# konstantineder/montecarlo-risk-engine

Measured on AMD Instinct MI355X. Metric: path-steps/sec at 1M paths x 250 steps; PV/CVA rel-error vs CPU ref, higher is better.
Workload: dtype f64

## Files before the change

montecarlo-risk-engine_amd/csrc/kf_lean.hip:

```cpp
#include <cstdlib>
#include <map>
#include <utility>

#include "kf_common.h"

namespace {

template <int NSLOT, int PPL>
__device__ __forceinline__ void lean_date_cva(const FastDateCvaLds* __restrict__ rp, const double (&reg)[PPL][2 * NSLOT], double (&cva)[PPL],
                                              const double* __restrict__ etab)
{
    const mcx_expq_coef ec = mcx_expq_load(mcx_region_zero());
    const FastDateCvaLds r = *rp;
    double xe[2 * PPL], ev[2 * PPL];
#pragma unroll
    for (int q = 0; q < PPL; ++q) {
        xe[2 * q] = fma(r.m_s1, reg[q][FDC_S_REG], fma(r.m_n1, reg[q][FDC_NI_REG], r.m_c0));
        xe[2 * q + 1] = fma(r.c_c1, reg[q][FDC_C_REG], r.c_c0);
    }
    mcx_exp_tab_n<2 * PPL>(xe, ev, etab, ec);
#pragma unroll
    for (int q = 0; q < PPL; ++q) {
        const double x = fma(r.x_d, reg[q][FDC_X_REG], r.x_a);
        double p = 0.0;
        p += fma(fma(r.row0[2], x, r.row0[1]), x, r.row0[0]);
        p += fma(fma(r.row1[2], x, r.row1[1]), x, r.row1[0]);
        const double w = r.m_b * ev[2 * q];
        const double cs = fma(r.c_b, ev[2 * q + 1], r.c_a);
        cva[q] = fma(fmax(p, 0.0), w * (1.0 - cs), cva[q]);
    }
}

template <int PPL>
__device__ __forceinline__ void philox4x32_10_cva(const uint32_t (&path_lo)[PPL], uint32_t path_hi, uint32_t step, uint32_t draw, uint64_t seed,
                                                  uint32_t (&o0)[PPL], uint32_t (&o1)[PPL], uint32_t (&o2)[PPL], uint32_t (&o3)[PPL])
{
    constexpr uint32_t M0 = 0xD2511F53u, M1 = 0xCD9E8D57u, W0 = 0x9E3779B9u, W1 = 0xBB67AE85u;
    uint32_t k0 = (uint32_t)seed, k1 = (uint32_t)(seed >> 32);
    uint32_t c0[PPL], c1[PPL], c2[PPL], c3[PPL];
    const uint64_t s1 = (uint64_t)M1 * step;
    const uint32_t hk = path_hi ^ k0;
    const uint32_t a0 = (uint32_t)(s1 >> 32) ^ hk, a1 = (uint32_t)s1;
    const uint32_t dk = draw ^ k1;
#pragma unroll
    for (int q = 0; q < PPL; ++q) {
        const uint64_t p0 = (uint64_t)M0 * path_lo[q];
        c2[q] = (uint32_t)(p0 >> 32) ^ dk;
        c3[q] = (uint32_t)p0;
    }
    k0 += W0; k1 += W1;
    const uint64_t s0 = (uint64_t)M0 * a0;
#pragma unroll
    for (int q = 0; q < PPL; ++q) {
        const uint64_t p1 = (uint64_t)M1 * c2[q];
        c0[q] = ((uint32_t)(p1 >> 32) ^ k0) ^ a1;
        c2[q] = (c3[q] ^ k1) ^ (uint32_t)(s0 >> 32);
        c1[q] = (uint32_t)p1;
    }
    k0 += W0; k1 += W1;
    const uint32_t x3 = (uint32_t)s0 ^ k1;
#pragma unroll
    for (int q = 0; q < PPL; ++q) {
        const uint64_t p0 = (uint64_t)M0 * c0[q];
        const uint64_t p1 = (uint64_t)M1 * c2[q];
        c0[q] = __builtin_amdgcn_bitop3_b32((uint32_t)(p1 >> 32), c1[q], k0, 0x96);
        c2[q] = (uint32_t)(p0 >> 32) ^ x3;
        c1[q] = (uint32_t)p1; c3[q] = (uint32_t)p0;
    }
    k0 += W0; k1 += W1;
#pragma unroll
    for (int r = 3; r < 10; ++r) {
#pragma unroll
        for (int q = 0; q < PPL; ++q) {
            const uint64_t p0 = (uint64_t)M0 * c0[q];
            const uint64_t p1 = (uint64_t)M1 * c2[q];
            const uint32_t n0 = __builtin_amdgcn_bitop3_b32((uint32_t)(p1 >> 32), c1[q], k0, 0x96);
            const uint32_t n2 = __builtin_amdgcn_bitop3_b32((uint32_t)(p0 >> 32), c3[q], k1, 0x96);
            c1[q] = (uint32_t)p1; c3[q] = (uint32_t)p0; c0[q] = n0; c2[q] = n2;
        }
        k0 += W0; k1 += W1;
    }
#pragma unroll
    for (int q = 0; q < PPL; ++q) { o0[q] = c0[q]; o1[q] = c1[q]; o2[q] = c2[q]; o3[q] = c3[q]; }
}

struct CvaDrawConst {
    double off52;
    double trig_scale;
};
__device__ __forceinline__ CvaDrawConst cva_draw_const_make()
{
    CvaDrawConst c;
    c.off52 = mcx_opaque_v(0x1.0p52 - 0.5); c.trig_scale = mcx_opaque_v(6.28318530717958647692 * 0x1.0p-53);
    return c;
}

template <int PPL, int BMB>
__device__ __forceinline__ bool cva_draw_pairs(uint64_t seed, const uint32_t (&path_lo)[PPL], uint32_t path_hi, uint32_t step, uint32_t draw,
                                               double (&z0)[PPL], double (&z1)[PPL], const double* __restrict__ tab,
                                               const mcx_bm_coef& C, const mcx_bm_vconst& vc, const CvaDrawConst& dc)
{
    static_assert(BMB >= 1 && BMB <= 20, "the funnel shift of the high word is by 11 + BMB < 32 bits");
    constexpr int N = 1 << BMB, LOG_TERMS = mcx_bm_shape<BMB>::LOG_TERMS;
    uint32_t w0[PPL], w1[PPL], w2[PPL], w3[PPL];
    philox4x32_10_cva<PPL>(path_lo, path_hi, step, draw, seed, w0, w1, w2, w3);
    double m[PPL], ed[PPL], ps[PPL], pc[PPL];
    int e[PPL];
    mcx_d2 tc[PPL], sc[PPL];
#pragma unroll
    for (int q = 0; q < PPL; ++q) {
        const double ua = u53(w0[q], w1[q], &vc);
        m[q] = __builtin_amdgcn_frexp_mant(ua);
        e[q] = __builtin_amdgcn_frexp_exp(ua);
        const int jl = (__double2hiint(m[q]) >> (20 - BMB)) & (N - 1);
        tc[q] = ((const mcx_d2*)tab)[jl];
        sc[q] = ((const mcx_d2*)(tab + 2 * N))[(int)(w3[q] >> (32 - BMB))];
    }
    __builtin_amdgcn_sched_barrier(0);
#pragma unroll
    for (int q = 0; q < PPL; ++q) {
        const uint32_t lo = __builtin_amdgcn_alignbit(w3[q], w2[q], 11);
        const uint32_t hi = __builtin_amdgcn_alignbit(0x43300000u >> (21 - BMB), w3[q] << BMB, 11 + BMB);
        const double v = __hiloint2double((int)hi, (int)lo) - dc.off52;
        const double d = fma(v, dc.trig_scale, vc.trig_off);
        const double d2 = d * d;
        double qs, qc;
        if constexpr (mcx_bm_shape<BMB>::TRIG_TERMS == 3) {
            qs = fma(fma(vc.sin_head, d2, C.c[7]), d2, C.c[6]);
            qc = fma(fma(vc.cos_head, d2, C.c[10]), d2, C.c[9]);
        } else {
            qs = fma(vc.sin_head, d2, C.c[6]);
            qc = fma(vc.cos_head, d2, C.c[9]);
        }
        ps[q] = fma(d * d2, qs, d);
        pc[q] = fma(d2, qc, 1.0);
        ed[q] = (double)e[q];
    }
    __builtin_amdgcn_sched_barrier(0);
    uint32_t top = 0;
#pragma unroll
    for (int q = 0; q < PPL; ++q) {
        const double s = fma(m[q], tc[q].x, 2.0);
        double p = vc.log_head;
#pragma unroll
        for (int k = LOG_TERMS - 2; k >= 0; --k) p = fma(p, s, C.c[k]);
        const double r2 = fma(ed[q], -2.0 * 6.93147180559945309417e-01, tc[q].y) + fma(s * s, p, s);
        const double r = mcx_sqrt_gp(r2);
        const double sn = fma(sc[q].x, pc[q], sc[q].y * ps[q]);
        const double cs = fma(-sc[q].x, ps[q], sc[q].y * pc[q]);
        z0[q] = r * cs;
        z1[q] = r * sn;
        top = w1[q] > top ? w1[q] : top;
    }
    return top == 0xffffffffu;
}

#define MCX_LEAN_WAVES 4
template <int NSLOT, int NZ, bool INJECT, int SIG, int PPL, bool SIMULATE, int DK = 0>
__global__ __launch_bounds__(MCX_BLOCK, MCX_LEAN_WAVES) void kf_lean(const FusedArgs)
{
    static_assert(DK == 0 || (SIG == SIG_VAS_CIR_E && SIMULATE && !INJECT), "the cva-date kernel simulates the Vasicek + CIR++ signature");
    constexpr int NREG = 2 * NSLOT;
    constexpr int TILE = MCX_BLOCK * PPL;
    extern __shared__ double lds[];
    KArgs& a0 = kargs_region(0);
    const int n_rec = a0.n_rec;
    const int64_t n = a0.k1.n;
    for (int q = threadIdx.x; q < 9 * n_rec; q += MCX_BLOCK) lds[q] = 0.0;
    FastDateCvaLds* const dlds = (FastDateCvaLds*)(lds + ((9 * n_rec + 1) & ~1));
    if constexpr (DK != 0) {
        const FastDateCva* __restrict__ dc = a0.cva_dates;
        const double* __restrict__ cf = a0.coeffs;
        const int n_dates = a0.n_dates;
        for (int q = threadIdx.x; q < 16 * n_dates; q += MCX_BLOCK) {
            const int t = q >> 4, e = q & 15;
            double v;
            if (e < FDC_HEAD) {
                v = ((const double*)(dc + t))[e];
            } else {
                const int off = e < FDC_HEAD + 3 ? dc[t].coeff_off0 : dc[t].coeff_off1;
                v = off >= 0 ? cf[off + (e - FDC_HEAD) % 3] : 0.0;
            }
            ((double*)dlds)[q] = v;
        }
    }
    constexpr int BMB = SIG == SIG_VAS_CIR_E ? 10 : 7;
    constexpr int BM = (INJECT || !SIMULATE) ? 0 : MCX_BM_LDS_DOUBLES_B(BMB);
    __shared__ double tab_lds[BM + MCX_EXP_LDS_DOUBLES];
    const double* tab = nullptr;
    const double* etab = tab_lds + BM;
    mcx_exp_tab_load(tab_lds + BM);
    if (BM) { mcx_bm_load<BMB>(tab_lds); tab = tab_lds; }
    __syncthreads();
    const int64_t tiles = (n + TILE - 1) / TILE;
    double n_block = 0.0;

    for (int64_t tile = blockIdx.x; tile < tiles; tile += gridDim.x) {
        const bool first_tile = tile == (int64_t)blockIdx.x;
        int64_t i[PPL];
        bool live[PPL];
        uint64_t path[PPL];
        double reg[PPL][NREG];
        double cfs[PPL], cva[PPL];
        int est[PPL];
        int n_init, n_steps;
        {
            KArgs& a = kargs_region(mcx_region_zero());
            const auto& k = a.k1;
#pragma unroll
            for (int q = 0; q < PPL; ++q) {
                const int64_t i_raw = tile * TILE + q * MCX_BLOCK + threadIdx.x;
                live[q] = i_raw < n;
                i[q] = live[q] ? i_raw : n - 1;
                path[q] = k.path_offset + (uint64_t)i[q];
                sim_init_state<NSLOT, SIG>(k, reg[q]);
                cfs[q] = 0.0; cva[q] = 0.0;
                est[q] = a.init_state[0];
            }
            const int64_t rest = n - tile * TILE;
            n_block += (double)(rest < TILE ? rest : TILE);
            n_init = k.n_initial_store; n_steps = k.n_steps;
        }
        if (SIMULATE) {
        int step = 0, t_init = 0;
#pragma unroll 1
        while (true) {
            const bool init = t_init < n_init;
            if (!init && step >= n_steps) break;
            int st = init ? t_init : -1;
            t_init += init ? 1 : 0;
            {
                const int zr0 = mcx_region_zero();
                const auto& k = kargs_region(zr0).k1;
                const uint64_t seed = k.seed;
                const mcx_bm_coef bc = mcx_bm_coef_load(zr0);
                const mcx_bm_vconst vc = mcx_bm_vconst_make<BMB>(bc);
                uint32_t path_hi = 0;
                CvaDrawConst dc = {};
                if constexpr (DK == 1) { path_hi = ((const MCX_KONST uint32_t*)&k.path_offset)[1]; dc = cva_draw_const_make(); }
#pragma unroll 1
                while (st < 0 && step < n_steps) {
                    if constexpr (SIG == SIG_GENERIC) {
#pragma unroll
                        for (int q = 0; q < PPL; ++q) sim_substep<NSLOT, NZ, INJECT, SIG, BMB, true>(k, step, path[q], i[q], reg[q], tab, seed, bc, &vc);
                        st = ldk(&k.steps[step].store_idx);
                    } else {
                        double zz[PPL][NZ], uu[PPL];
                        bool rare = false;
                        const StepData<NSLOT, NZ> sdat = sim_step_load<NSLOT, NZ, SIG>(k, step);
                        __builtin_amdgcn_sched_barrier(0);
                        if constexpr (INJECT) {
#pragma unroll
                            for (int q = 0; q < PPL; ++q) sim_draw<NZ, true, SIG, BMB>(k, step, path[q], i[q], zz[q], uu[q], tab, seed, bc, &vc);
                        } else if constexpr (DK == 1) {
                            static_assert(NZ == 2, "one Philox block per path and sub-step");
                            uint32_t plo[PPL];
                            double za[PPL], zb[PPL];
#pragma unroll
                            for (int q = 0; q < PPL; ++q) plo[q] = (uint32_t)path[q];
                            rare = cva_draw_pairs<PPL, BMB>(seed, plo, path_hi, (uint32_t)step, 0u, za, zb, tab, bc, vc, dc);
#pragma unroll
                            for (int q = 0; q < PPL; ++q) { zz[q][0] = za[q]; zz[q][1] = zb[q]; uu[q] = 0.0; }
                        } else {
                            uint32_t st_q[PPL];
#pragma unroll
                            for (int q = 0; q < PPL; ++q) st_q[q] = (uint32_t)step;
                            rare = sim_draw_n<PPL, NZ, SIG, BMB>(k, st_q, path, zz, uu, tab, seed, bc, vc);
                        }
                        if (!INJECT && __builtin_expect(__any(rare), 0)) {
                            if constexpr (DK == 1) {
#pragma unroll
                                for (int q = 0; q < PPL; ++q)
                                    sim_draw<NZ, false, SIG, BMB, true>(k, step, ((uint64_t)path_hi << 32) | (uint32_t)path[q], i[q], zz[q], uu[q], tab, seed, bc, &vc);
                            } else {
#pragma unroll
                                for (int q = 0; q < PPL; ++q) sim_draw<NZ, false, SIG, BMB, true>(k, step, path[q], i[q], zz[q], uu[q], tab, seed, bc, &vc);
                            }
                        }
#pragma unroll
                        for (int q = 0; q < PPL; ++q) st = sim_apply_loaded<NSLOT, NZ, SIG, true>(k, sdat, reg[q], zz[q], uu[q]);
                    }
                    ++step;
                }
            }
            if (st >= 0) {
                if constexpr (DK != 0) lean_date_cva<NSLOT, PPL>(dlds + st, reg, cva, etab);
                else lean_date<NSLOT, SIG, PPL, true>(st, i, live, first_tile, lds, reg, cfs, cva, est, etab);
            }
        }
        } else {
            auto load_row = [&](int t, double (&dst)[PPL][NREG]) {
                const auto& k = kargs_region(0).k1;
                const int D = k.n_state;
#pragma unroll
                for (int q = 0; q < PPL; ++q)
#pragma unroll
                    for (int sl = 0; sl < NSLOT; ++sl) {
                        const bool bs = sig_kind(SIG, sl) >= 0 ? sig_is_bs(SIG, sl) : (k.slots[sl].kind == MCX_MODEL_BS);
                        const int c = k.slots[sl].state_off;
                        dst[q][2 * sl] = k.paths[((int64_t)t * D + c) * k.ld + i[q]];
                        dst[q][2 * sl + 1] = bs ? 0.0 : k.paths[((int64_t)t * D + c + 1) * k.ld + i[q]];
                    }
            };
            const int n_dates = kargs_region(0).n_dates;
            double bufb[PPL][NREG];
            load_row(0, reg);
            load_row(n_dates > 1 ? 1 : 0, bufb);
#pragma unroll 1
            for (int t = 0; t < n_dates; t += 2) {
                lean_date<NSLOT, SIG, PPL, false>(t, i, live, first_tile, lds, reg, cfs, cva, est, etab);
                if (t + 2 < n_dates) load_row(t + 2, reg);
                if (t + 1 < n_dates) {
                    lean_date<NSLOT, SIG, PPL, false>(t + 1, i, live, first_tile, lds, bufb, cfs, cva, est, etab);
                    if (t + 3 < n_dates) load_row(t + 3, bufb);
                }
            }
        }
        {
            KArgs& a = kargs_region(mcx_region_zero());
#pragma unroll
            for (int q = 0; q < PPL; ++q) if (a.cfs && live[q]) a.cfs[i[q]] = cfs[q];
            if (a.rec_pv[0] >= 0) lean_record<PPL>(cfs, live, a.rec_pv[0], n_rec, first_tile, lds);
            if (a.rec_cva[0] >= 0) {
                const double lgd = a.lgd[0];
                double cc[PPL];
#pragma unroll
                for (int q = 0; q < PPL; ++q) cc[q] = cva[q] * lgd;
                lean_record<PPL>(cc, live, a.rec_cva[0], n_rec, first_tile, lds);
            }
        }
    }
    __syncthreads();
    for (int r = threadIdx.x; r < n_rec; r += MCX_BLOCK) {
        double s1 = 0.0, s2 = 0.0;
        for (int w = 0; w < 4; ++w) { s1 += lds[n_rec + (w * n_rec + r) * 2]; s2 += lds[n_rec + (w * n_rec + r) * 2 + 1]; }
        double* dst = a0.partials + ((int64_t)blockIdx.x * n_rec + r) * 4;
        dst[0] = n_block; dst[1] = lds[r]; dst[2] = s1; dst[3] = s2;
    }
}

template <int NSLOT, int NZ, int SIG, int PPL>
int launch_lean_shape(const FusedArgs& a, int full_steps, int n_cu, bool inject, bool simulate, hipStream_t s)
{
    const int64_t tiles = (a.k1.n + MCX_BLOCK * PPL - 1) / (MCX_BLOCK * PPL);
    const size_t lds = sizeof(double) * (size_t)((9 * a.n_rec + 1) & ~1);
    const size_t lds_cva = lds + sizeof(FastDateCvaLds) * (size_t)a.n_dates;
    auto residency = [&](auto kernel, size_t bytes) {
        thread_local std::map<std::pair<const void*, size_t>, int> cache;
        const auto key = std::make_pair((const void*)kernel, bytes);
        auto it = cache.find(key);
        if (it == cache.end()) {
            int per_cu = 0;
            if (hipOccupancyMaxActiveBlocksPerMultiprocessor(&per_cu, kernel, MCX_BLOCK, bytes) != hipSuccess || per_cu < 1) per_cu = 1;
            it = cache.emplace(key, per_cu < MCX_LEAN_WAVES ? per_cu : MCX_LEAN_WAVES).first;
        }
        return (int64_t)it->second * n_cu;
    };
    auto sized = [&](int64_t resident) {
        if (tiles <= resident) return (int)tiles;
        const int64_t per = (tiles + resident - 1) / resident;
        return (int)((tiles + per - 1) / per);
    };
    int grid;
    if (!simulate) {
        auto kern = kf_lean<NSLOT, NZ, false, SIG, PPL, false>;
        grid = sized(residency(kern, lds));
        hipLaunchKernelGGL(kern, dim3(grid), dim3(MCX_BLOCK), lds, s, a);
    } else if (inject) {
        auto kern = kf_lean<NSLOT, NZ, true, SIG, PPL, true>;
        grid = sized(residency(kern, lds));
        hipLaunchKernelGGL(kern, dim3(grid), dim3(MCX_BLOCK), lds, s, a);
    } else {
        auto kern = kf_lean<NSLOT, NZ, false, SIG, PPL, true>;
        const int64_t resident = residency(kern, lds);
        if constexpr (SIG == SIG_VAS_CIR_E) {
            auto kern_cva = kf_lean<NSLOT, NZ, false, SIG, 2, true, 1>;
            auto kern_cva_thin = kf_lean<NSLOT, NZ, false, SIG, PPL, true, 2>;
            const bool one_high_word = ((a.k1.path_offset + (uint64_t)(a.k1.n - 1)) >> 32) == (a.k1.path_offset >> 32);
            if (a.cva_dates && one_high_word) {
                grid = sized(resident);
                if (PPL == 2 && grid >= resident) {
                    if (residency(kern_cva, lds_cva) >= resident) {
                        hipLaunchKernelGGL(kern_cva, dim3(grid), dim3(MCX_BLOCK), lds_cva, s, a);
                        return grid;
                    }
                } else if (residency(kern_cva_thin, lds_cva) >= resident) {
                    hipLaunchKernelGGL(kern_cva_thin, dim3(grid), dim3(MCX_BLOCK), lds_cva, s, a);
                    return grid;
                }
            }
        }
        grid = sized(resident);
        FusedArgs g = a;
        g.k1.n_steps = full_steps;
        hipLaunchKernelGGL(kern, dim3(grid), dim3(MCX_BLOCK), lds, s, g);
    }
    return grid;
}

template <int NSLOT, int NZ, int SIG>
void launch_lean(const FusedArgs& a, int full_steps, int n_cu, bool inject, bool simulate, hipStream_t s, int* grid_out)
{
    constexpr int PPL = (SIG == SIG_GENERIC && NSLOT >= 2) ? 1 : 2;
#ifdef MCX_LEAN_AB
    if (simulate && !inject) {
        const char* sh = getenv("MCX_LEAN_SHAPE");
        const int code = sh ? atoi(sh) : 0;
        if (code == 11) { *grid_out = launch_lean_shape<NSLOT, NZ, SIG, 1>(a, full_steps, n_cu, inject, simulate, s); return; }
        if (code == 21) { *grid_out = launch_lean_shape<NSLOT, NZ, SIG, 2>(a, full_steps, n_cu, inject, simulate, s); return; }
    }
#endif
    const int64_t full_tiles = (a.k1.n + MCX_BLOCK * PPL - 1) / (MCX_BLOCK * PPL);
    if (PPL == 2 && simulate && !inject && full_tiles < (int64_t)2 * n_cu) {
        *grid_out = launch_lean_shape<NSLOT, NZ, SIG, 1>(a, full_steps, n_cu, inject, simulate, s);
        return;
    }
    *grid_out = launch_lean_shape<NSLOT, NZ, SIG, PPL>(a, full_steps, n_cu, inject, simulate, s);
}

}

int mcx_launch_kf_lean(const FusedArgs& a, const mcx_sim_desc& sd, int n_cu, bool inject, bool simulate, hipStream_t s)
{
    int grid = -1;
#ifdef MCX_LEAN_ONE_SIG
    if (mcx_sim_signature(sd) == SIG_VAS_CIR_E) launch_lean<2, 2, SIG_VAS_CIR_E>(a, sd.n_steps, n_cu, inject, simulate, s, &grid);
#else
    mcx_dispatch_signature<4>(sd, [&](auto nslot, auto nz, auto sig) {
        launch_lean<decltype(nslot)::value, decltype(nz)::value, decltype(sig)::value>(a, sd.n_steps, n_cu, inject, simulate, s, &grid);
    });
#endif
    return grid;
}
```

Before: 309.9 billion.

## Hoist step-invariant Philox rounds per tile and split a dedicated CVA loop

```diff
diff --git a/montecarlo-risk-engine_amd/csrc/cva_words.h b/montecarlo-risk-engine_amd/csrc/cva_words.h
--- /dev/null
+++ b/montecarlo-risk-engine_amd/csrc/cva_words.h
@@ -0,0 +1,31 @@
+#pragma once
+#include <cstdint>
+
+#if defined(__HIPCC__)
+#define CVA_W_FN __host__ __device__ __forceinline__
+#else
+#define CVA_W_FN static inline
+#endif
+
+CVA_W_FN double cva_w_hilo(uint32_t hi, uint32_t lo)
+{
+    const uint64_t b = ((uint64_t)hi << 32) | lo;
+    double x;
+    __builtin_memcpy(&x, &b, 8);
+    return x;
+}
+CVA_W_FN uint32_t cva_w_hi(double x)
+{
+    uint64_t b;
+    __builtin_memcpy(&b, &x, 8);
+    return (uint32_t)(b >> 32);
+}
+
+#define CVA_W_C54H (0x1.0p-54 - 0.5)
+CVA_W_FN double cva_w_low_part(uint32_t lo, double c54h)
+{
+    return cva_w_hilo(0x3fe00000u, lo >> 11) + c54h;
+}
+
+template <int BMB>
+CVA_W_FN uint32_t cva_w_log_byte_offset(uint32_t hi_ua) { return (hi_ua >> (16 - BMB)) & (((1u << BMB) - 1u) << 4); }
diff --git a/montecarlo-risk-engine_amd/csrc/kf_lean.hip b/montecarlo-risk-engine_amd/csrc/kf_lean.hip
--- a/montecarlo-risk-engine_amd/csrc/kf_lean.hip
+++ b/montecarlo-risk-engine_amd/csrc/kf_lean.hip
@@ -3,6 +3,7 @@
 #include <utility>
 
 #include "kf_common.h"
+#include "cva_words.h"
 
 namespace {
 
@@ -31,33 +32,48 @@
     }
 }
 
+
 template <int PPL>
-__device__ __forceinline__ void philox4x32_10_cva(const uint32_t (&path_lo)[PPL], uint32_t path_hi, uint32_t step, uint32_t draw, uint64_t seed,
+struct CvaTileWords {
+    uint32_t c0k[PPL];
+    uint32_t c1[PPL];
+    uint32_t c2k[PPL];
+};
+template <int PPL>
+__device__ __forceinline__ CvaTileWords<PPL> philox_cva_tile(const uint32_t (&path_lo)[PPL], uint32_t draw, uint64_t seed)
+{
+    constexpr uint32_t M0 = 0xD2511F53u, M1 = 0xCD9E8D57u, W0 = 0x9E3779B9u, W1 = 0xBB67AE85u;
+    const uint32_t k0 = (uint32_t)seed, k1 = (uint32_t)(seed >> 32);
+    const uint32_t dk = draw ^ k1;
+    CvaTileWords<PPL> t;
+#pragma unroll
+    for (int q = 0; q < PPL; ++q) {
+        const uint64_t p0 = (uint64_t)M0 * path_lo[q];
+        const uint64_t p1 = (uint64_t)M1 * ((uint32_t)(p0 >> 32) ^ dk);
+        t.c0k[q] = (uint32_t)(p1 >> 32) ^ (k0 + W0);
+        t.c1[q] = (uint32_t)p1;
+        t.c2k[q] = (uint32_t)p0 ^ (k1 + W1);
+    }
+    return t;
+}
+
+template <int PPL>
+__device__ __forceinline__ void philox4x32_10_cva(const CvaTileWords<PPL>& t, uint32_t path_hi, uint32_t step, uint64_t seed,
                                                   uint32_t (&o0)[PPL], uint32_t (&o1)[PPL], uint32_t (&o2)[PPL], uint32_t (&o3)[PPL])
 {
     constexpr uint32_t M0 = 0xD2511F53u, M1 = 0xCD9E8D57u, W0 = 0x9E3779B9u, W1 = 0xBB67AE85u;
     uint32_t k0 = (uint32_t)seed, k1 = (uint32_t)(seed >> 32);
     uint32_t c0[PPL], c1[PPL], c2[PPL], c3[PPL];
     const uint64_t s1 = (uint64_t)M1 * step;
-    const uint32_t hk = path_hi ^ k0;
-    const uint32_t a0 = (uint32_t)(s1 >> 32) ^ hk, a1 = (uint32_t)s1;
-    const uint32_t dk = draw ^ k1;
-#pragma unroll
-    for (int q = 0; q < PPL; ++q) {
-        const uint64_t p0 = (uint64_t)M0 * path_lo[q];
-        c2[q] = (uint32_t)(p0 >> 32) ^ dk;
-        c3[q] = (uint32_t)p0;
-    }
-    k0 += W0; k1 += W1;
+    const uint32_t a0 = (uint32_t)(s1 >> 32) ^ (path_hi ^ k0), a1 = (uint32_t)s1;
     const uint64_t s0 = (uint64_t)M0 * a0;
 #pragma unroll
     for (int q = 0; q < PPL; ++q) {
-        const uint64_t p1 = (uint64_t)M1 * c2[q];
-        c0[q] = ((uint32_t)(p1 >> 32) ^ k0) ^ a1;
-        c2[q] = (c3[q] ^ k1) ^ (uint32_t)(s0 >> 32);
-        c1[q] = (uint32_t)p1;
-    }
-    k0 += W0; k1 += W1;
+        c0[q] = t.c0k[q] ^ a1;
+        c2[q] = t.c2k[q] ^ (uint32_t)(s0 >> 32);
+        c1[q] = t.c1[q];
+    }
+    k0 += 2 * W0; k1 += 2 * W1;
     const uint32_t x3 = (uint32_t)s0 ^ k1;
 #pragma unroll
     for (int q = 0; q < PPL; ++q) {
@@ -87,33 +103,56 @@
 struct CvaDrawConst {
     double off52;
     double trig_scale;
+    double c54h;
 };
 __device__ __forceinline__ CvaDrawConst cva_draw_const_make()
 {
     CvaDrawConst c;
     c.off52 = mcx_opaque_v(0x1.0p52 - 0.5); c.trig_scale = mcx_opaque_v(6.28318530717958647692 * 0x1.0p-53);
+    c.c54h = mcx_opaque_v(CVA_W_C54H);
     return c;
 }
 
+template <int BMB>
+__device__ __forceinline__ mcx_bm_vconst cva_vconst_make(const mcx_bm_coef& C)
+{
+    using SH = mcx_bm_shape<BMB>;
+    mcx_bm_vconst v;
+    v.c54 = mcx_opaque_v(0x1.0p-54);
+    v.s53 = 0x1.0p-53; v.s32 = 0x1.0p-32;
+    v.log_head = mcx_opaque_v(C.c[SH::LOG_TERMS - 1]);
+    v.sin_head = mcx_opaque_v(C.c[5 + SH::TRIG_TERMS]);
+    v.cos_head = mcx_opaque_v(C.c[8 + SH::TRIG_TERMS]);
+    v.trig_off = mcx_opaque_v(-3.14159265358979323846 / (double)(1 << BMB));
+    return v;
+}
+template <int DK>
+__device__ __forceinline__ mcx_bm_vconst cva_run_vconst(mcx_bm_vconst v)
+{
+    if (DK != 1) v.s53 = mcx_opaque_s(0x1.0p-53);
+    v.s32 = mcx_opaque_s(0x1.0p-32);
+    return v;
+}
+__device__ __forceinline__ uint32_t cva_rare_word(uint32_t x) { asm volatile("" : "+v"(x)); return x; }
+
 template <int PPL, int BMB>
-__device__ __forceinline__ bool cva_draw_pairs(uint64_t seed, const uint32_t (&path_lo)[PPL], uint32_t path_hi, uint32_t step, uint32_t draw,
+__device__ __forceinline__ bool cva_draw_pairs(uint64_t seed, const CvaTileWords<PPL>& tw, uint32_t path_hi, uint32_t step,
                                                double (&z0)[PPL], double (&z1)[PPL], const double* __restrict__ tab,
                                                const mcx_bm_coef& C, const mcx_bm_vconst& vc, const CvaDrawConst& dc)
 {
     static_assert(BMB >= 1 && BMB <= 20, "the funnel shift of the high word is by 11 + BMB < 32 bits");
     constexpr int N = 1 << BMB, LOG_TERMS = mcx_bm_shape<BMB>::LOG_TERMS;
     uint32_t w0[PPL], w1[PPL], w2[PPL], w3[PPL];
-    philox4x32_10_cva<PPL>(path_lo, path_hi, step, draw, seed, w0, w1, w2, w3);
+    philox4x32_10_cva<PPL>(tw, path_hi, step, seed, w0, w1, w2, w3);
     double m[PPL], ed[PPL], ps[PPL], pc[PPL];
     int e[PPL];
     mcx_d2 tc[PPL], sc[PPL];
 #pragma unroll
     for (int q = 0; q < PPL; ++q) {
-        const double ua = u53(w0[q], w1[q], &vc);
+        const double ua = fma((double)w1[q], vc.s32, cva_w_low_part(w0[q], dc.c54h));
         m[q] = __builtin_amdgcn_frexp_mant(ua);
         e[q] = __builtin_amdgcn_frexp_exp(ua);
-        const int jl = (__double2hiint(m[q]) >> (20 - BMB)) & (N - 1);
-        tc[q] = ((const mcx_d2*)tab)[jl];
+        tc[q] = *(const mcx_d2*)((const char*)tab + cva_w_log_byte_offset<BMB>(cva_w_hi(ua)));
         sc[q] = ((const mcx_d2*)(tab + 2 * N))[(int)(w3[q] >> (32 - BMB))];
     }
     __builtin_amdgcn_sched_barrier(0);
@@ -194,6 +233,10 @@
     __syncthreads();
     const int64_t tiles = (n + TILE - 1) / TILE;
     double n_block = 0.0;
+    mcx_bm_vconst vck = {};
+    CvaDrawConst dck = {};
+    if constexpr (DK != 0) vck = cva_vconst_make<BMB>(mcx_bm_coef_load(mcx_region_zero()));
+    if constexpr (DK == 1) dck = cva_draw_const_make();
 
     for (int64_t tile = blockIdx.x; tile < tiles; tile += gridDim.x) {
         const bool first_tile = tile == (int64_t)blockIdx.x;
@@ -221,7 +264,62 @@
             n_block += (double)(rest < TILE ? rest : TILE);
             n_init = k.n_initial_store; n_steps = k.n_steps;
         }
-        if (SIMULATE) {
+        if constexpr (DK != 0) {
+            uint32_t plo[PPL];
+#pragma unroll
+            for (int q = 0; q < PPL; ++q) plo[q] = (uint32_t)path[q];
+            CvaTileWords<PPL> tw = {};
+            if constexpr (DK == 1) tw = philox_cva_tile<PPL>(plo, 0u, kargs_region(mcx_region_zero()).k1.seed);
+#pragma unroll 1
+            for (int t = 0; t < n_init; ++t) lean_date_cva<NSLOT, PPL>(dlds + t, reg, cva, etab);
+            int step = 0;
+#pragma unroll 1
+            while (step < n_steps) {
+                int st;
+                {
+                    const int zr0 = mcx_region_zero();
+                    const auto& k = kargs_region(zr0).k1;
+                    const uint64_t seed = k.seed;
+                    const mcx_bm_coef bc = mcx_bm_coef_load(zr0);
+                    const mcx_bm_vconst vc = cva_run_vconst<DK>(vck);
+                    uint32_t path_hi = 0;
+                    if constexpr (DK == 1) path_hi = ((const MCX_KONST uint32_t*)&k.path_offset)[1];
+#pragma unroll 1
+                    do {
+                        double zz[PPL][NZ], uu[PPL];
+                        bool rare;
+                        const StepData<NSLOT, NZ> sdat = sim_step_load<NSLOT, NZ, SIG>(k, step);
+                        __builtin_amdgcn_sched_barrier(0);
+                        if constexpr (DK == 1) {
+                            static_assert(NZ == 2, "one Philox block per path and sub-step");
+                            double za[PPL], zb[PPL];
+                            rare = cva_draw_pairs<PPL, BMB>(seed, tw, path_hi, (uint32_t)step, za, zb, tab, bc, vc, dck);
+#pragma unroll
+                            for (int q = 0; q < PPL; ++q) { zz[q][0] = za[q]; zz[q][1] = zb[q]; uu[q] = 0.0; }
+                        } else {
+                            uint32_t st_q[PPL];
+#pragma unroll
+                            for (int q = 0; q < PPL; ++q) st_q[q] = (uint32_t)step;
+                            rare = sim_draw_n<PPL, NZ, SIG, BMB>(k, st_q, path, zz, uu, tab, seed, bc, vc);
+                        }
+                        if (__builtin_expect(__any(rare), 0)) {
+                            if constexpr (DK == 1) {
+#pragma unroll
+                                for (int q = 0; q < PPL; ++q)
+                                    sim_draw<NZ, false, SIG, BMB, true>(k, step, ((uint64_t)path_hi << 32) | cva_rare_word(plo[q]), i[q], zz[q], uu[q], tab, seed, bc, &vc);
+                            } else {
+#pragma unroll
+                                for (int q = 0; q < PPL; ++q) sim_draw<NZ, false, SIG, BMB, true>(k, step, path[q], i[q], zz[q], uu[q], tab, seed, bc, &vc);
+                            }
+                        }
+#pragma unroll
+                        for (int q = 0; q < PPL; ++q) st = sim_apply_loaded<NSLOT, NZ, SIG, true>(k, sdat, reg[q], zz[q], uu[q]);
+                        ++step;
+                    } while (st < 0 && step < n_steps);
+                }
+                if (st >= 0) lean_date_cva<NSLOT, PPL>(dlds + st, reg, cva, etab);
+            }
+        } else if (SIMULATE) {
         int step = 0, t_init = 0;
 #pragma unroll 1
         while (true) {
@@ -235,9 +333,6 @@
                 const uint64_t seed = k.seed;
                 const mcx_bm_coef bc = mcx_bm_coef_load(zr0);
                 const mcx_bm_vconst vc = mcx_bm_vconst_make<BMB>(bc);
-                uint32_t path_hi = 0;
-                CvaDrawConst dc = {};
-                if constexpr (DK == 1) { path_hi = ((const MCX_KONST uint32_t*)&k.path_offset)[1]; dc = cva_draw_const_make(); }
 #pragma unroll 1
                 while (st < 0 && step < n_steps) {
                     if constexpr (SIG == SIG_GENERIC) {
@@ -252,15 +347,6 @@
                         if constexpr (INJECT) {
 #pragma unroll
                             for (int q = 0; q < PPL; ++q) sim_draw<NZ, true, SIG, BMB>(k, step, path[q], i[q], zz[q], uu[q], tab, seed, bc, &vc);
-                        } else if constexpr (DK == 1) {
-                            static_assert(NZ == 2, "one Philox block per path and sub-step");
-                            uint32_t plo[PPL];
-                            double za[PPL], zb[PPL];
-#pragma unroll
-                            for (int q = 0; q < PPL; ++q) plo[q] = (uint32_t)path[q];
-                            rare = cva_draw_pairs<PPL, BMB>(seed, plo, path_hi, (uint32_t)step, 0u, za, zb, tab, bc, vc, dc);
-#pragma unroll
-                            for (int q = 0; q < PPL; ++q) { zz[q][0] = za[q]; zz[q][1] = zb[q]; uu[q] = 0.0; }
                         } else {
                             uint32_t st_q[PPL];
 #pragma unroll
@@ -268,14 +354,8 @@
                             rare = sim_draw_n<PPL, NZ, SIG, BMB>(k, st_q, path, zz, uu, tab, seed, bc, vc);
                         }
                         if (!INJECT && __builtin_expect(__any(rare), 0)) {
-                            if constexpr (DK == 1) {
-#pragma unroll
-                                for (int q = 0; q < PPL; ++q)
-                                    sim_draw<NZ, false, SIG, BMB, true>(k, step, ((uint64_t)path_hi << 32) | (uint32_t)path[q], i[q], zz[q], uu[q], tab, seed, bc, &vc);
-                            } else {
-#pragma unroll
-                                for (int q = 0; q < PPL; ++q) sim_draw<NZ, false, SIG, BMB, true>(k, step, path[q], i[q], zz[q], uu[q], tab, seed, bc, &vc);
-                            }
+#pragma unroll
+                            for (int q = 0; q < PPL; ++q) sim_draw<NZ, false, SIG, BMB, true>(k, step, path[q], i[q], zz[q], uu[q], tab, seed, bc, &vc);
                         }
 #pragma unroll
                         for (int q = 0; q < PPL; ++q) st = sim_apply_loaded<NSLOT, NZ, SIG, true>(k, sdat, reg[q], zz[q], uu[q]);
@@ -283,10 +363,7 @@
                     ++step;
                 }
             }
-            if (st >= 0) {
-                if constexpr (DK != 0) lean_date_cva<NSLOT, PPL>(dlds + st, reg, cva, etab);
-                else lean_date<NSLOT, SIG, PPL, true>(st, i, live, first_tile, lds, reg, cfs, cva, est, etab);
-            }
+            if (st >= 0) lean_date<NSLOT, SIG, PPL, true>(st, i, live, first_tile, lds, reg, cfs, cva, est, etab);
         }
         } else {
             auto load_row = [&](int t, double (&dst)[PPL][NREG]) {
```

New measurement: 324.0 billion, median of 6. 4.5% higher.
